# EnricoMiccoli/nodal

Measured on AMD Instinct MI355X. Metric: circuits_per_sec, higher is better.
Workload: dtype f64; 1 GPU; cfg3: grid(1000) 1e6 nodes, sparse CSR path; n=999999, nnz=4995995, parallelism=one GPU

## Files before the change

### nodal_amd/csrc/knobs.h

```cpp
#pragma once
#include <stdint.h>
#include <stdlib.h>

#include <optional>

namespace knob {

struct Present {
    const char *name;
    bool now() const { return getenv(name) != nullptr; }
};
struct OnUnless0 {
    const char *name;
    bool now() const { const char *e = getenv(name); return !(e && atoi(e) == 0); }
};
struct OffUnlessNon0 {
    const char *name;
    bool now() const { const char *e = getenv(name); return e && atoi(e) != 0; }
};
struct OnIfSet0 {
    const char *name;
    bool now() const { const char *e = getenv(name); return e != nullptr && atoi(e) == 0; }
};
struct Level {
    const char *name;
    int now() const {
        const char *e = getenv(name);
        if (!e) return 0;
        const int v = atoi(e);
        return v > 1 ? v : 1;
    }
};
struct Int {
    const char *name;
    int dflt;
    int now() const { const char *e = getenv(name); return e ? atoi(e) : dflt; }
};
struct Int64 {
    const char *name;
    int64_t dflt;
    int64_t now() const { const char *e = getenv(name); return e ? atoll(e) : dflt; }
};
struct Double {
    const char *name;
    double dflt;
    double now() const { const char *e = getenv(name); return e ? atof(e) : dflt; }
};
struct IntIfSet {
    const char *name;
    std::optional<int> now() const { const char *e = getenv(name); return e ? std::optional<int>(atoi(e)) : std::nullopt; }
};
struct Int64IfSet {
    const char *name;
    std::optional<int64_t> now() const { const char *e = getenv(name); return e ? std::optional<int64_t>(atoll(e)) : std::nullopt; }
};
struct DoubleIfSet {
    const char *name;
    std::optional<double> now() const { const char *e = getenv(name); return e ? std::optional<double>(atof(e)) : std::nullopt; }
};
struct Text {
    const char *name;
    const char *now() const { return getenv(name); }
};

inline constexpr Present TRACE{"NODAL_TRACE"};
inline constexpr Level POISON{"NODAL_POISON"};
inline constexpr Present NOFILL{"NODAL_NOFILL"};
inline constexpr Present NANCHECK{"NODAL_NANCHECK"};
inline constexpr Double WAIT_TIMEOUT_S{"NODAL_WAIT_TIMEOUT_S", 60.0};
inline constexpr Text STREAM_PRIORITY{"NODAL_STREAM_PRIORITY"};
inline constexpr IntIfSet EXTRA_STREAMS{"NODAL_EXTRA_STREAMS"};
inline constexpr IntIfSet HOST_THREADS{"NODAL_HOST_THREADS"};
inline constexpr IntIfSet CSV_CHUNKS{"NODAL_CSV_CHUNKS"};
inline constexpr OnUnless0 FOLD_STREAM{"NODAL_FOLD_STREAM"};
inline constexpr OffUnlessNon0 COUNT_LDS{"NODAL_COUNT_LDS"};
inline constexpr IntIfSet DENSE_BLOCKINV{"NODAL_DENSE_BLOCKINV"};
inline constexpr IntIfSet GJ_SCALAR{"NODAL_GJ_SCALAR"};
inline constexpr OnUnless0 GJ_DPP{"NODAL_GJ_DPP"};
inline constexpr OnUnless0 BI_SYM{"NODAL_BI_SYM"};
inline constexpr OnIfSet0 BI_MASKED{"NODAL_BI_MASKED"};
inline constexpr Int PANEL_CUS{"NODAL_PANEL_CUS", 32};
inline constexpr Int64 BI_UNMASK_ROWS{"NODAL_BI_UNMASK_ROWS", 0};
inline constexpr OnUnless0 BI_EARLY_COPY{"NODAL_BI_EARLY_COPY"};
inline constexpr Int BI_FIRST_BLOCKS{"NODAL_BI_FIRST_BLOCKS", 2};
inline constexpr Text BI_SWITCH{"NODAL_BI_SWITCH"};
inline constexpr Text BI_SWITCH2{"NODAL_BI_SWITCH2"};
inline constexpr Text BI_WIDTH{"NODAL_BI_WIDTH"};
inline constexpr IntIfSet GEPP_PANEL{"NODAL_GEPP_PANEL"};
inline constexpr Int GEPP_MAX{"NODAL_GEPP_MAX", 1280};
inline constexpr Present GEPP_PROBE{"NODAL_GEPP_PROBE"};
inline constexpr Int64IfSet FCG_MAXIT{"NODAL_FCG_MAXIT"};
inline constexpr OnUnless0 FCG_HOST_SUM{"NODAL_FCG_HOST_SUM"};
inline constexpr Double FCG_LOOK{"NODAL_FCG_LOOK", 0.75};
inline constexpr OnUnless0 LOWDEG{"NODAL_LOWDEG"};
inline constexpr IntIfSet LOWDEG_SHARE{"NODAL_LOWDEG_SHARE"};
inline constexpr Int64 LOWDEG_MIN{"NODAL_LOWDEG_MIN", 32};
inline constexpr Present SPARSE_FORCE_DIRECT{"NODAL_SPARSE_FORCE_DIRECT"};
inline constexpr Present SPARSE_CHILD_DIRECT{"NODAL_SPARSE_CHILD_DIRECT"};
inline constexpr OnUnless0 SAGG{"NODAL_SAGG"};
inline constexpr OnUnless0 SA_REUSE{"NODAL_SA_REUSE"};
inline constexpr OnUnless0 SA_FORK{"NODAL_SA_FORK"};
inline constexpr Double SA_SPREAD{"NODAL_SA_SPREAD", 16.0};
inline constexpr Double SA_SHARE{"NODAL_SA_SHARE", 0.9};
inline constexpr IntIfSet SA_MIS{"NODAL_SA_MIS"};
inline constexpr Text SA_OMEGA_P{"NODAL_SA_OMEGA_P"};
inline constexpr Double SA_PADSLACK{"NODAL_SA_PADSLACK", 1.3};
inline constexpr OnUnless0 SA_D16{"NODAL_SA_D16"};
inline constexpr Int SA_GG{"NODAL_SA_GG", 40};
inline constexpr Int64 SA_GCAP{"NODAL_SA_GCAP", 16384};
inline constexpr Int SA_GROWS{"NODAL_SA_GROWS", 4};
inline constexpr OnUnless0 SA_GDYN{"NODAL_SA_GDYN"};
inline constexpr Int SA_GLIST{"NODAL_SA_GLIST", 1024};
inline constexpr Int SA_GSEG{"NODAL_SA_GSEG", 4};
inline constexpr Text SA_NU{"NODAL_SA_NU"};
inline constexpr Int SA_KCYCLE{"NODAL_SA_KCYCLE", 1};
inline constexpr Int SA_KLEVELS{"NODAL_SA_KLEVELS", 1};
inline constexpr OnUnless0 SA_KFREEZE{"NODAL_SA_KFREEZE"};
inline constexpr OnUnless0 SA_FUSE_DIR{"NODAL_SA_FUSE_DIR"};
inline constexpr OffUnlessNon0 SA_GRAPH{"NODAL_SA_GRAPH"};
inline constexpr Text SA_FOLD_POST{"NODAL_SA_FOLD_POST"};
inline constexpr OffUnlessNon0 SA_FOLD_CHECK{"NODAL_SA_FOLD_CHECK"};
inline constexpr OnUnless0 SA_FOLD_VISIT{"NODAL_SA_FOLD_VISIT"};
inline constexpr Int64 SA_VISIT_CAP{"NODAL_SA_VISIT_CAP", 16777216};
inline constexpr OffUnlessNon0 SA_VISIT_CHECK{"NODAL_SA_VISIT_CHECK"};
inline constexpr OnUnless0 SA_RESTRICT_B{"NODAL_SA_RESTRICT_B"};
inline constexpr OffUnlessNon0 SA_RESTRICT_CHECK{"NODAL_SA_RESTRICT_CHECK"};
inline constexpr OnUnless0 SA_TAIL_DENSE{"NODAL_SA_TAIL_DENSE"};
inline constexpr OffUnlessNon0 SA_TAIL_CHECK{"NODAL_SA_TAIL_CHECK"};
inline constexpr Int SA_TAIL_NU{"NODAL_SA_TAIL_NU", 3};
inline constexpr Present TAIL_PROBE{"NODAL_TAIL_PROBE"};
inline constexpr IntIfSet AMG_PASSES0{"NODAL_AMG_PASSES0"};
inline constexpr IntIfSet AMG_PASSES1{"NODAL_AMG_PASSES1"};
inline constexpr IntIfSet AMG_SWEEPS0{"NODAL_AMG_SWEEPS0"};
inline constexpr IntIfSet AMG_BLOCK{"NODAL_AMG_BLOCK"};
inline constexpr DoubleIfSet AMG_THETA{"NODAL_AMG_THETA"};
inline constexpr Present AMG_KEEP_DENSE{"NODAL_AMG_KEEP_DENSE"};
inline constexpr Present AMG_NOTAIL{"NODAL_AMG_NOTAIL"};
inline constexpr IntIfSet AMG_KMAX{"NODAL_AMG_KMAX"};
inline constexpr OnUnless0 PAIRS_BLOCK{"NODAL_PAIRS_BLOCK"};
inline constexpr OnUnless0 PAIRS_FUNCTIONAL{"NODAL_PAIRS_FUNCTIONAL"};
inline constexpr Int PAIRS_DIRECT{"NODAL_PAIRS_DIRECT", -1};
inline constexpr Int64 PAIRS_DIRECT_MIN{"NODAL_PAIRS_DIRECT_MIN", 256};
inline constexpr Double MULTI_BAR{"NODAL_MULTI_BAR", 1e-14};
inline constexpr IntIfSet PRESOLVE{"NODAL_PRESOLVE"};
inline constexpr OnUnless0 PRESOLVE_KEEP{"NODAL_PRESOLVE_KEEP"};
inline constexpr IntIfSet FGMRES_WINDOW{"NODAL_FGMRES_WINDOW"};
inline constexpr Text DIRECT_NB{"NODAL_DIRECT_NB"};
inline constexpr Int DIRECT_LANES{"NODAL_DIRECT_LANES", 4};
inline constexpr DoubleIfSet DIRECT_MAX_GB{"NODAL_DIRECT_MAX_GB"};
inline constexpr IntIfSet DIRECT_BIG_DIM{"NODAL_DIRECT_BIG_DIM"};
inline constexpr OnUnless0 DIRECT_FRONT_LDS{"NODAL_DIRECT_FRONT_LDS"};
inline constexpr Int DIRECT_LDS_BS{"NODAL_DIRECT_LDS_BS", 64};
inline constexpr OnUnless0 DIRECT_PANEL_REGS{"NODAL_DIRECT_PANEL_REGS"};
inline constexpr OnUnless0 DIRECT_BATCHED{"NODAL_DIRECT_BATCHED"};
inline constexpr OnUnless0 DIRECT_WAVE{"NODAL_DIRECT_WAVE"};
inline constexpr Present DIRECT_LEVELS{"NODAL_DIRECT_LEVELS"};
inline constexpr OnUnless0 DIRECT_SUPER{"NODAL_DIRECT_SUPER"};
inline constexpr OnUnless0 DIRECT_APPLY_STEPPED{"NODAL_DIRECT_APPLY_STEPPED"};
inline constexpr OnUnless0 DIRECT_PEEL{"NODAL_DIRECT_PEEL"};
inline constexpr Int ND_DEPTH{"NODAL_ND_DEPTH", 4};
inline constexpr Int64 ND_PAR{"NODAL_ND_PAR", 20000};
inline constexpr Present SLU_DEBUG{"SLU_DEBUG"};

}
```

### nodal_amd/csrc/sagg.hip

```cpp
#include <hip/hip_ext.h>

#include <atomic>
#include <type_traits>

#include "galerkin_groups.h"
#include "group.h"

int grounded_flags(nodal_ctx *h, uint8_t *flags_dev);

namespace {

using grp::TB;
constexpr int PW = 4;
constexpr int ACAP = 64;
constexpr int RCAP = 96;
constexpr int RCAP_SMALL = 512;
constexpr int RCAP_SMALL_ROWS = 16384;
inline int rcap_for(int64_t nc) { return nc <= RCAP_SMALL_ROWS ? RCAP_SMALL : RCAP; }
constexpr int W0_MAX = 32;
constexpr int COARSEST = 64;
constexpr int MAX_LEVELS = 12;
constexpr int MIS_ROUNDS = 6;
constexpr int TAIL_MAX_N = 1024;
constexpr int TAIL_LEVELS = 6;
constexpr int TAIL_LDS_BUDGET = 150 * 1024;
constexpr int APAD = 32;
constexpr int DOT_BLOCKS = 1024;
#ifndef NODAL_SA_OMEGA
#define NODAL_SA_OMEGA 0.85
#endif
constexpr double OMEGA = NODAL_SA_OMEGA;
constexpr double OMEGA_P = 0.70;
constexpr double OMEGA_P_COARSE = 0.85;
using cyc_t = nodal_cyc_t;

inline unsigned grid_for(int64_t n, unsigned cap = 8192) {
    int64_t g = (n + TB - 1) / TB;
    if (g < 1) g = 1;
    if (g >= 64) g = (g + 7) & ~(int64_t)7;
    return (unsigned)(g > cap ? cap : g);
}
inline int64_t pad64(int64_t n) { return (n + 63) & ~(int64_t)63; }
inline size_t align256(size_t x) { return (x + 255) & ~(size_t)255; }

__device__ __forceinline__ unsigned xcd_block() {
    const unsigned g = gridDim.x, b = blockIdx.x;
    return (g & 7u) ? b : (b & 7u) * (g >> 3) + (b >> 3);
}


struct Ell {
    int64_t n = 0, ld = 0;
    int32_t width = 0;
    const int32_t *col = nullptr;
    const int16_t *dcol = nullptr;
    const double *val = nullptr;
    const float *valf = nullptr;
    const int32_t *len = nullptr;
};

enum { ST_MAXLEN = 0, ST_GRADED = 1, ST_BADDIAG = 2, ST_OVERFLOW = 3, ST_NNZ = 4, ST_UNASSIGNED = 5,
       ST_MAXR = 6, ST_NC = 7 ,
       ST_FARCOL = 8 ,
       ST_FOLDMISS = 9 ,
       ST_VISITMISS = 10 ,
       ST_RESTRICTMISS = 11 ,
       ST_COUNT = 12 };

struct SLevel {
    int64_t n = 0, ld = 0, nc = 0;
    int32_t width = 0;
    int32_t maxlen = 0;
    int32_t wfix = 0;
    int64_t nnz = 0;
    DevBuf acol, aval, alen, dinv;
    DevBuf adcol;
    bool d16 = false;
    DevBuf agg, pcol, pval;
    DevBuf rcol, rval, rlen;
    int64_t rld = 0;
    DevBuf vec, part, gflag;
    DevBuf avalf, pvalf, rvalf;
    DevBuf wcol, wval, wlen;
    int32_t wslots = 0;
    bool fold_want = false, fold = false;
    DevBuf p2col, p2val, p2len, d2;
    bool visit_want = false, visit = false;
    DevBuf wtstart, wtcol, wtval, wtsrc;
// ... 132 lines not shown
        m = max(m, bstat[i]);
        t += bstat[BSTAT_MAX + i];
    }
    atomicMax(&s_max, m);
    atomicAdd(&s_sum, t);
    __syncthreads();
    if (threadIdx.x == 0) {
        if (slot_max >= 0) stats[slot_max] = s_max;
        if (slot_sum >= 0) stats[slot_sum] = s_sum;
    }
}

__global__ __launch_bounds__(TB) void row_stats(int64_t n, const int32_t *__restrict__ indptr,
                                                const int32_t *__restrict__ indices,
                                                const double *__restrict__ data, double share, double spread,
                                                bool general, unsigned long long *__restrict__ stats,
                                                uint32_t *__restrict__ bstat) {
    int32_t mlen = 0;
    uint32_t graded = 0, bad = 0, far = 0;
    for (int64_t i = (int64_t)xcd_block() * TB + threadIdx.x; i < n; i += (int64_t)gridDim.x * TB) {
        const int32_t e0 = indptr[i], e1 = indptr[i + 1];
        mlen = max(mlen, e1 - e0);
        double d = 0.0, mx = 0.0, mn = 1e300;
        for (int32_t e = e0; e < e1; ++e) {
            const double v = data[e];
            const int64_t dc = (int64_t)indices[e] - i;
            if (dc > 32767 || dc < -32767) far = 1;
            if (indices[e] == (int32_t)i) d = v;
            else if (v != 0.0) {
                mx = fmax(mx, fabs(v));
                mn = fmin(mn, fabs(v));
                if (v > 0.0 && !general) bad = 1;
            }
        }
        if (!(d > 0.0)) bad = 1;
        graded += (d > 0.0 && (mx > share * d || mx > spread * mn)) ? 1u : 0u;
    }
    __shared__ unsigned int s_len, s_graded, s_bad;
    if (threadIdx.x == 0) s_len = s_graded = s_bad = 0;
    __syncthreads();
    atomicMax(&s_len, (unsigned)mlen);
    if (graded) atomicAdd(&s_graded, graded);
    if (bad) atomicOr(&s_bad, 1u);
    if (far) atomicOr(&s_bad, 2u);
    __syncthreads();
    if (threadIdx.x == 0) {
        bstat[blockIdx.x] = s_len;
        bstat[BSTAT_MAX + blockIdx.x] = s_graded;
        if (s_bad & 1u) atomicOr(&stats[ST_BADDIAG], 1ull);
        if (s_bad & 2u) stats[ST_FARCOL] = 1ull;
    }
}

__global__ __launch_bounds__(TB) void csr_to_ell(int64_t n, int64_t ld, const int32_t *__restrict__ indptr,
                                                 const int32_t *__restrict__ indices,
                                                 const double *__restrict__ data, int32_t *__restrict__ col,
                                                 double *__restrict__ val, float *__restrict__ valf,
                                                 int32_t *__restrict__ len, double *__restrict__ dinv, int32_t wpad,
                                                 int16_t *__restrict__ dcol) {
    for (int64_t i = (int64_t)xcd_block() * TB + threadIdx.x; i < n; i += (int64_t)gridDim.x * TB) {
        const int32_t e0 = indptr[i], e1 = indptr[i + 1];
        double d = 1.0;
        for (int32_t e = e0; e < e1; ++e) {
            const int32_t c = indices[e];
            const double v = data[e];
            col[(int64_t)(e - e0) * ld + i] = c;
            if (dcol) dcol[(int64_t)(e - e0) * ld + i] = (int16_t)(c - (int32_t)i);
            val[(int64_t)(e - e0) * ld + i] = v;
            valf[(int64_t)(e - e0) * ld + i] = (float)v;
            if (c == (int32_t)i) d = v;
        }
        for (int32_t s = e1 - e0; s < wpad; ++s) {
            col[(int64_t)s * ld + i] = (int32_t)i;
            if (dcol) dcol[(int64_t)s * ld + i] = 0;
            val[(int64_t)s * ld + i] = 0.0;
            valf[(int64_t)s * ld + i] = 0.0f;
        }
        len[i] = e1 - e0;
        dinv[i] = 1.0 / d;
    }
}


__device__ __forceinline__ uint32_t hash30(uint32_t x) {
    x ^= x >> 16;
    x *= 0x7feb352du;
    x ^= x >> 15;
    x *= 0x846ca68bu;
    x ^= x >> 16;
    return x & 0x3fffffffu;
}

__global__ __launch_bounds__(TB) void mis_init(int64_t n, uint32_t *__restrict__ T) {
    for (int64_t i = (int64_t)xcd_block() * TB + threadIdx.x; i < n; i += (int64_t)gridDim.x * TB)
        T[i] = (1u << 30) | hash30((uint32_t)i);
}

template <int NB>
__device__ __forceinline__ uint32_t nbr_max_batch(const Ell &A, const uint32_t *__restrict__ v, int64_t i, int32_t l, int32_t s0,
                                                  uint32_t best) {
    int32_t c[NB];
#pragma unroll
    for (int u = 0; u < NB; ++u) c[u] = A.col[(int64_t)(s0 + u < l ? s0 + u : 0) * A.ld + i];
    uint32_t t[NB];
#pragma unroll
    for (int u = 0; u < NB; ++u) t[u] = v[c[u]];
#pragma unroll
    for (int u = 0; u < NB; ++u) best = t[u] > best ? t[u] : best;
    return best;
}
__device__ __forceinline__ uint32_t nbr_max(const Ell &A, const uint32_t *__restrict__ v, int64_t i, int32_t l, uint32_t best) {
    if (l <= 5) return nbr_max_batch<5>(A, v, i, l, 0, best);
    for (int32_t s0 = 0; s0 < l; s0 += 8) best = nbr_max_batch<8>(A, v, i, l, s0, best);
    return best;
}

__global__ __launch_bounds__(TB) void mis_max(Ell A, const uint32_t *__restrict__ v, uint32_t *__restrict__ m) {
    for (int64_t i = (int64_t)xcd_block() * TB + threadIdx.x; i < A.n; i += (int64_t)gridDim.x * TB)
        m[i] = nbr_max(A, v, i, A.len[i], v[i]);
}

__global__ __launch_bounds__(TB) void mis_update(Ell A, uint32_t *__restrict__ T, const uint32_t *__restrict__ m1) {
    for (int64_t i = (int64_t)xcd_block() * TB + threadIdx.x; i < A.n; i += (int64_t)gridDim.x * TB) {
        const uint32_t own = T[i];
        if ((own >> 30) != 1) continue;
        const uint32_t best = nbr_max(A, m1, i, A.len[i], m1[i]);
        if (best == own) T[i] = own | (2u << 30);
        else if ((best >> 30) == 3) T[i] = 0;
    }
}

__global__ __launch_bounds__(TB) void mis_count(int64_t n, const uint32_t *__restrict__ T,
                                                unsigned long long *__restrict__ out) {
    uint32_t left = 0;
    for (int64_t i = (int64_t)xcd_block() * TB + threadIdx.x; i < n; i += (int64_t)gridDim.x * TB)
        left += (T[i] >> 30) == 1 ? 1u : 0u;
#pragma unroll
    for (int off = 32; off > 0; off >>= 1) left += __shfl_down(left, off, 64);
    if ((threadIdx.x & 63) == 0 && left) atomicAdd(out, (unsigned long long)left);
}

__global__ __launch_bounds__(TB) void mis_flag_roots(Ell A, const uint32_t *__restrict__ T,
                                                     uint32_t *__restrict__ flag) {
    for (int64_t i = (int64_t)xcd_block() * TB + threadIdx.x; i <= A.n; i += (int64_t)gridDim.x * TB) {
        uint32_t f = 0;
        if (i < A.n) {
            const uint32_t own = T[i];
            if ((own >> 30) == 3) f = 1;
            else if ((own >> 30) == 1) {
                bool near = false;
                const int32_t l = A.len[i];
                for (int32_t s = 0; s < l; ++s) near = near || (T[A.col[(int64_t)s * A.ld + i]] >> 30) == 3;
                f = near ? 0u : 1u;
            }
        }
        flag[i] = f;
    }
}

constexpr int64_t MIS_SMALL_MAX = 1024;
__global__ __launch_bounds__(1024) void mis_small(Ell A, uint32_t *__restrict__ T, uint32_t *__restrict__ M,
                                                  uint32_t *__restrict__ flag, int rounds) {
    const int64_t n = A.n;
    for (int64_t i = threadIdx.x; i < n; i += 1024) T[i] = (1u << 30) | hash30((uint32_t)i);
    __syncthreads();
    for (int r = 0; r < rounds; ++r) {
        for (int64_t i = threadIdx.x; i < n; i += 1024) {
            uint32_t best = T[i];
            const int32_t l = A.len[i];
            for (int32_t s = 0; s < l; ++s) {
                const uint32_t t = T[A.col[(int64_t)s * A.ld + i]];
                best = t > best ? t : best;
            }
            M[i] = best;
        }
        __syncthreads();
        for (int64_t i = threadIdx.x; i < n; i += 1024) {
            const uint32_t own = T[i];
            if ((own >> 30) != 1) continue;
            uint32_t best = M[i];
            const int32_t l = A.len[i];
            for (int32_t s = 0; s < l; ++s) {
                const uint32_t t = M[A.col[(int64_t)s * A.ld + i]];
                best = t > best ? t : best;
            }
            if (best == own) T[i] = own | (2u << 30);
            else if ((best >> 30) == 3) T[i] = 0;
        }
        __syncthreads();
    }
    for (int64_t i = threadIdx.x; i <= n; i += 1024) {
        uint32_t f = 0;
        if (i < n) {
            const uint32_t own = T[i];
            if ((own >> 30) == 3) f = 1;
            else if ((own >> 30) == 1) {
                bool near = false;
                const int32_t l = A.len[i];
                for (int32_t s = 0; s < l; ++s) near = near || (T[A.col[(int64_t)s * A.ld + i]] >> 30) == 3;
                f = near ? 0u : 1u;
            }
        }
        flag[i] = f;
    }
}

__global__ __launch_bounds__(TB) void assign_near(Ell A, const uint32_t *__restrict__ T,
                                                  const uint32_t *__restrict__ flag,
                                                  const uint32_t *__restrict__ id, int32_t *__restrict__ agg1) {
    for (int64_t i = (int64_t)xcd_block() * TB + threadIdx.x; i < A.n; i += (int64_t)gridDim.x * TB) {
        int32_t a = -1;
        if (flag[i]) a = (int32_t)id[i];
        else {
            uint32_t best = 0;
            const int32_t l = A.len[i];
            auto batch = [&](auto NBc, int32_t s0) {
                constexpr int NB = decltype(NBc)::value;
                int32_t c[NB];
#pragma unroll
                for (int u = 0; u < NB; ++u) c[u] = A.col[(int64_t)(s0 + u < l ? s0 + u : 0) * A.ld + i];
                uint32_t fl[NB], tt[NB], idd[NB];
#pragma unroll
                for (int u = 0; u < NB; ++u) {
                    fl[u] = flag[c[u]];
                    tt[u] = T[c[u]];
                    idd[u] = id[c[u]];
                }
#pragma unroll
                for (int u = 0; u < NB; ++u) {
                    if (s0 + u >= l || c[u] == (int32_t)i || !fl[u]) continue;
                    const uint32_t t = tt[u] | (3u << 30);
                    if (t > best) { best = t; a = (int32_t)idd[u]; }
                }
            };
            if (l <= 5) batch(std::integral_constant<int, 5>{}, 0);
            else for (int32_t s0 = 0; s0 < l; s0 += 8) batch(std::integral_constant<int, 8>{}, s0);
        }
        agg1[i] = a;
    }
}

__global__ __launch_bounds__(TB) void assign_far(Ell A, const int32_t *__restrict__ agg1, int32_t *__restrict__ agg,
                                                 unsigned long long *__restrict__ stats) {
    for (int64_t i = (int64_t)xcd_block() * TB + threadIdx.x; i < A.n; i += (int64_t)gridDim.x * TB) {
        int32_t a = agg1[i];
        if (a < 0) {
            double bw = -1.0;
            const int32_t l = A.len[i];
            auto batch = [&](auto NBc, int32_t s0) {
                constexpr int NB = decltype(NBc)::value;
                int32_t c[NB];
                double w[NB];
#pragma unroll
                for (int u = 0; u < NB; ++u) {
                    const int64_t at = (int64_t)(s0 + u < l ? s0 + u : 0) * A.ld + i;
                    c[u] = A.col[at];
                    w[u] = fabs(A.val[at]);
                }
                int32_t aj[NB];
#pragma unroll
                for (int u = 0; u < NB; ++u) aj[u] = agg1[c[u]];
#pragma unroll
                for (int u = 0; u < NB; ++u) {
                    if (s0 + u >= l || c[u] == (int32_t)i || aj[u] < 0) continue;
                    if (w[u] > bw) { bw = w[u]; a = aj[u]; }
                }
            };
            if (l <= 5) batch(std::integral_constant<int, 5>{}, 0);
            else for (int32_t s0 = 0; s0 < l; s0 += 8) batch(std::integral_constant<int, 8>{}, s0);
            if (a < 0) stats[ST_UNASSIGNED] = 1;
        }
        agg[i] = a;
    }
}

__global__ __launch_bounds__(TB) void build_P(Ell A, const double *__restrict__ dinv,
                                              const int32_t *__restrict__ agg, int32_t *__restrict__ pcol,
                                              double *__restrict__ pval, float *__restrict__ pvalf, double omega_p) {
    for (int64_t i = (int64_t)xcd_block() * TB + threadIdx.x; i < A.n; i += (int64_t)gridDim.x * TB) {
        int32_t c[PW];
        double v[PW];
#pragma unroll
        for (int k = 0; k < PW; ++k) { c[k] = -1; v[k] = 0.0; }
        const int32_t own = agg[i];
        c[0] = own;
        v[0] = 1.0;
        const double wd = omega_p * dinv[i];
        const int32_t l = A.len[i];
        for (int32_t s = 0; s < l; ++s) {
            const int32_t J = agg[A.col[(int64_t)s * A.ld + i]];
            const double t = -wd * A.val[(int64_t)s * A.ld + i];
            bool placed = false;
#pragma unroll
            for (int k = 0; k < PW; ++k) {
                if (!placed && c[k] == J) { v[k] += t; placed = true; }
            }
#pragma unroll
            for (int k = 1; k < PW; ++k) {
                if (!placed && c[k] < 0) { c[k] = J; v[k] = t; placed = true; }
            }
            if (!placed) v[0] += t;
        }
#pragma unroll
        for (int k = 0; k < PW; ++k) {
            pcol[(int64_t)k * A.ld + i] = c[k];
            pval[(int64_t)k * A.ld + i] = v[k];
            pvalf[(int64_t)k * A.ld + i] = (float)v[k];
        }
    }
}

template <bool LEN>
struct TKey { static constexpr int SHIFT = LEN ? 6 : 2; };
template <bool LEN = false>
__global__ __launch_bounds__(TB) void r_count(int64_t n, int64_t ld, const int32_t *__restrict__ pcol,
                                              uint32_t *__restrict__ cnt, uint32_t *__restrict__ place,
                                              const int32_t *__restrict__ len = nullptr) {
    for (int64_t i = (int64_t)xcd_block() * TB + threadIdx.x; i < n; i += (int64_t)gridDim.x * TB) {
        if constexpr (LEN) {
            const int32_t m = len[i];
            for (int32_t k = 0; k < m; ++k)
                place[(int64_t)k * ld + i] = atomicAdd(&cnt[pcol[(int64_t)k * ld + i]], 1u);
        } else {
#pragma unroll
            for (int k = 0; k < PW; ++k) {
                const int32_t J = pcol[(int64_t)k * ld + i];
                if (J >= 0) place[(int64_t)k * ld + i] = atomicAdd(&cnt[J], 1u);
            }
        }
    }
}
template <bool LEN = false>
__global__ __launch_bounds__(TB) void r_fill(int64_t n, int64_t ld, const int32_t *__restrict__ pcol,
                                             const uint32_t *__restrict__ rstart, const uint32_t *__restrict__ place,
                                             uint64_t *__restrict__ keys, const int32_t *__restrict__ len = nullptr,
                                             uint32_t keycap = 0, int64_t nc = 0) {
    if constexpr (LEN) {
        if (rstart[nc] > keycap) return;
    }
    for (int64_t i = (int64_t)xcd_block() * TB + threadIdx.x; i < n; i += (int64_t)gridDim.x * TB) {
        if constexpr (LEN) {
            const int32_t m = len[i];
            for (int32_t k = 0; k < m; ++k)
                keys[rstart[pcol[(int64_t)k * ld + i]] + place[(int64_t)k * ld + i]] =
                    ((uint64_t)i << TKey<true>::SHIFT) | (uint64_t)k;
        } else {
#pragma unroll
            for (int k = 0; k < PW; ++k) {
                const int32_t J = pcol[(int64_t)k * ld + i];
                if (J >= 0) keys[rstart[J] + place[(int64_t)k * ld + i]] = ((uint64_t)i << 2) | (uint64_t)k;
            }
        }
    }
}
__global__ __launch_bounds__(TB) void r_to_ell(int64_t nc, int64_t rld, const uint32_t *__restrict__ rstart,
// ... 904 lines not shown
        return f;
    }();
    return s;
}
bool fold_wanted(int level, int64_t n) {
    if (level > 0 && n <= TAIL_MAX_N) return false;
    const FoldSetting &f = fold_setting();
    switch (f.mode) {
    case 1: return false;
    case 2: return true;
    case 3: return (f.mask >> level & 1u) != 0;
    default: return n <= FOLD_MAX_ROWS;
    }
}
void decide_folds(SHierarchy *H, const unsigned long long *hs, bool trace) {
    for (int k = 0; k < H->nlev; ++k) {
        SLevel *L = H->pool[k];
        const bool runs_cycle = k + 1 < H->nlev && (H->tail < 0 || k < H->tail);
        const bool miss = hs[(size_t)k * ST_COUNT + ST_FOLDMISS] != 0;
        L->fold = L->fold_want && runs_cycle && !miss;
        if (trace && L->fold_want && runs_cycle)
            fprintf(stderr, "[sagg] level %d (%lld rows): first post-smoothing sweep %s\n", k, (long long)L->n,
                    miss ? "NOT folded: a row of A P lacks a column of its P row (no stored diagonal)"
                         : "folded into the prolongation");
        const bool wide = hs[(size_t)k * ST_COUNT + ST_VISITMISS] != 0;
        L->visit = L->visit_want && L->fold && !wide;
        if (trace && L->visit_want)
            fprintf(stderr, "[sagg] level %d (%lld rows): visit %s\n", k, (long long)L->n,
                    L->visit ? "in three launches" : "NOT in three launches: W missing, or a row of P2 beyond its slots");
        const unsigned long long over = hs[(size_t)k * ST_COUNT + ST_RESTRICTMISS] |
                                        (H->sym_valid ? H->sym_stats[(size_t)k * ST_COUNT + ST_RESTRICTMISS] : 0ull);
        L->restrict_b = L->restrict_want && L->fold && !L->visit && !over;
        if (trace && L->restrict_want && runs_cycle)
            fprintf(stderr, "[sagg] level %d (%lld rows): restriction %s\n", k, (long long)L->n,
                    L->restrict_b ? "from b beside the residual launch"
                                  : over ? "NOT from b: a row of W^T beyond the per-row sort, or more entries than its arrays hold"
                                         : "NOT from b: W missing, or the level visits in three launches");
    }
}

void apply_nu_knob(SHierarchy *H);
constexpr int WT_AVG = 16;
bool restrict_wanted(SHierarchy *H, int l, const SLevel *L) {
    static const bool on = knob::SA_RESTRICT_B.now();
    if (!on || l < 1 || H->general || !L->fold_want || (int64_t)L->wslots * L->ld >= (1ll << 31)) return false;
    apply_nu_knob(H);
    return H->nu[l < 2 ? l : 2] == 1;
}
int reserve_wt(nodal_ctx *h, SHierarchy *H, SLevel *L, int64_t nc) {
    const int64_t cap = (int64_t)(L->wslots < WT_AVG ? L->wslots : WT_AVG) * L->n;
    L->wtcap = cap;
    NODAL_HIP_TRY(h, L->wtstart.reserve(align256((size_t)(nc + 1) * 4) + 256));
    NODAL_HIP_TRY(h, L->wtcol.reserve((size_t)cap * 4 + 64));
    NODAL_HIP_TRY(h, L->wtval.reserve((size_t)cap * 4 + 64));
    NODAL_HIP_TRY(h, L->wtsrc.reserve((size_t)cap * 4 + 64));
    NODAL_HIP_TRY(h, H->wt_keys.reserve((size_t)cap * 8 + 64));
    NODAL_HIP_TRY(h, H->wt_scratch.reserve(align256(scan_tmp_bytes(nc + 1)) + (size_t)L->wslots * L->ld * 4 + 64));
    return NODAL_OK;
}
int build_wt(nodal_ctx *h, SHierarchy *H, int l) {
    hipStream_t st = h->stream;
    SLevel *L = H->pool[l];
    const int64_t n = L->n, ld = L->ld, nc = L->nc;
    const uint32_t cap = (uint32_t)L->wtcap;
    uint32_t *wtstart = L->wtstart.as<uint32_t>();
    char *sc = H->wt_scratch.as<char>();
    uint32_t *place = reinterpret_cast<uint32_t *>(sc + align256(scan_tmp_bytes(nc + 1)));
    uint64_t *keys = H->wt_keys.as<uint64_t>();
    const int32_t *wcol = L->wcol.as<int32_t>(), *wlen = L->wlen.as<int32_t>();
    NODAL_HIP_TRY(h, hipMemsetAsync(wtstart, 0, align256((size_t)(nc + 1) * 4) + 256, st));
    r_count<true><<<grid_for(n), TB, 0, st>>>(n, ld, wcol, wtstart, place, wlen);
    NODAL_HIP_TRY(h, hipGetLastError());
    NODAL_TRY(scan_exclusive_u32(h, wtstart, wtstart, nc + 1, nullptr, sc));
    r_fill<true><<<grid_for(n), TB, 0, st>>>(n, ld, wcol, wtstart, place, keys, wlen, cap, nc);
    r_sort_short<<<grid_for(nc), TB, 0, st>>>(wtstart, keys, nc, cap);
    r_sort_medium<<<(unsigned)(nc < 8192 ? nc : 8192), 64, 0, st>>>(wtstart, keys, nc, cap);
    wt_pack<<<grid_for(nc * 64), TB, 0, st>>>(nc, wtstart, keys, ld, L->wval.as<float>(), cap, L->wtcol.as<int32_t>(),
                                             L->wtval.as<float>(), L->wtsrc.as<int32_t>(),
                                             H->stats.as<unsigned long long>() + (size_t)l * ST_COUNT);
    NODAL_HIP_TRY(h, hipGetLastError());
    return NODAL_OK;
}

int build_level(nodal_ctx *h, SHierarchy *H, int l, unsigned long long *hs, bool *declined, bool *stop) {
    hipStream_t st = h->stream;
    SLevel *L = H->level(l);
    const int64_t n = L->n, ld = L->ld;
    Ell A = L->A();
    A.width = L->maxlen;
    unsigned long long *dstats = H->stats.as<unsigned long long>();

    NODAL_HIP_TRY(h, H->mis_t.reserve((size_t)n * 8 + 64));
    NODAL_HIP_TRY(h, H->mis_m.reserve((size_t)n * 8 + 64));
    NODAL_HIP_TRY(h, H->mis_flag.reserve((size_t)(n + 1) * 4 + 64));
    NODAL_HIP_TRY(h, H->mis_id.reserve((size_t)(n + 1) * 4 + 64 + scan_tmp_bytes(n + 1)));
    NODAL_HIP_TRY(h, H->agg1.reserve((size_t)n * 4 + 64));
    NODAL_HIP_TRY(h, L->agg.reserve((size_t)n * 4 + 64));
    NODAL_HIP_TRY(h, H->cursor.reserve((MIS_ROUNDS + 2) * 8 + 64));
    uint32_t *T = H->mis_t.as<uint32_t>(), *M = H->mis_m.as<uint32_t>();
    uint32_t *flag = H->mis_flag.as<uint32_t>(), *id = H->mis_id.as<uint32_t>();
    unsigned long long *cnt = H->cursor.as<unsigned long long>();
    void *scan_tmp = H->mis_id.as<char>() + (((size_t)(n + 1) * 4 + 63) & ~(size_t)63);

    const unsigned g = grid_for(n);
    static const bool trace_mis = knob::TRACE.now();
    if (trace_mis) NODAL_HIP_TRY(h, hipMemsetAsync(cnt, 0, (MIS_ROUNDS + 2) * 8, st));
    static const int mis_rounds = std::min(MIS_ROUNDS, std::max(1, knob::SA_MIS.now().value_or(MIS_ROUNDS)));
    if (n <= MIS_SMALL_MAX && !trace_mis) {
        mis_small<<<1, 1024, 0, st>>>(A, T, M, flag, mis_rounds);
    } else {
        mis_init<<<g, TB, 0, st>>>(n, T);
        for (int r = 0; r < mis_rounds; ++r) {
            mis_max<<<g, TB, 0, st>>>(A, T, M);
            mis_update<<<g, TB, 0, st>>>(A, T, M);
            if (trace_mis) mis_count<<<g, TB, 0, st>>>(n, T, cnt + r + 1);
        }
        mis_flag_roots<<<grid_for(n + 1), TB, 0, st>>>(A, T, flag);
    }
    NODAL_HIP_TRY(h, hipGetLastError());
    NODAL_TRY(scan_exclusive_u32(h, flag, id, n + 1, reinterpret_cast<uint32_t *>(dstats + (size_t)l * ST_COUNT + ST_NC),
                                 scan_tmp));
    NODAL_HIP_TRY(h, hipMemcpyAsync(hs, dstats, (size_t)MAX_LEVELS * ST_COUNT * 8, hipMemcpyDeviceToHost, st));
    unsigned long long hcnt[MIS_ROUNDS + 1] = {0};
    if (trace_mis) NODAL_HIP_TRY(h, hipMemcpyAsync(hcnt, cnt, sizeof hcnt, hipMemcpyDeviceToHost, st));
    if (!H->ev_copy) NODAL_HIP_TRY(h, hipEventCreateWithFlags(&H->ev_copy, hipEventDisableTiming));
    NODAL_HIP_TRY(h, hipEventRecord(H->ev_copy, st));
    NODAL_HIP_TRY(h, L->pcol.reserve((size_t)PW * ld * 4 + 64));
    NODAL_HIP_TRY(h, L->pval.reserve((size_t)PW * ld * 8 + 64));
    NODAL_HIP_TRY(h, L->pvalf.reserve((size_t)PW * ld * 4 + 64));
    assign_near<<<g, TB, 0, st>>>(A, T, flag, id, H->agg1.as<int32_t>());
    assign_far<<<g, TB, 0, st>>>(A, H->agg1.as<int32_t>(), L->agg.as<int32_t>(), dstats + (size_t)l * ST_COUNT);
    build_P<<<g, TB, 0, st>>>(A, L->dinv.as<double>(), L->agg.as<int32_t>(), L->pcol.as<int32_t>(),
                             L->pval.as<double>(), L->pvalf.as<float>(), omega_p(l));
    NODAL_HIP_TRY(h, hipGetLastError());
    NODAL_WAIT_EVENT(h, H->ev_copy, st);
    if (trace_mis) {
        fprintf(stderr, "[sagg] level %d: undecided after each MIS round:", l);
        for (int r = 1; r <= MIS_ROUNDS; ++r) fprintf(stderr, " %llu", hcnt[r]);
        fprintf(stderr, "\n");
    }
    const int64_t nc = (int64_t)(hs[(size_t)l * ST_COUNT + ST_NC] & 0xffffffffull);
    if (l > 0) {
        const unsigned long long *s = hs + (size_t)l * ST_COUNT;
        L->maxlen = (int32_t)s[ST_MAXLEN];
        L->nnz = (int64_t)s[ST_NNZ];
        A.width = L->maxlen;
        if (s[ST_OVERFLOW] || s[ST_BADDIAG] || hs[(size_t)(l - 1) * ST_COUNT + ST_OVERFLOW] ||
            hs[(size_t)(l - 1) * ST_COUNT + ST_UNASSIGNED]) {
            *declined = true;
            return NODAL_OK;
        }
    }
    if (nc >= n || L->maxlen <= 1) {
        *stop = true;
        return NODAL_OK;
    }
    if ((nc * 2 > n && n > 4096) || nc < 1) {
        *declined = true;
        return NODAL_OK;
    }
    L->nc = nc;

    static const bool fork_allowed = knob::SA_FORK.now();
    if (H->aux && !nodal_extra_streams_ok(h) && nodal_calls_in_flight() <= 1) {
        NODAL_WAIT_STREAM(h, H->aux);
        (void)hipStreamDestroy(H->aux);
        H->aux = nullptr;
        H->aux_tried = false;
    }
    if (fork_allowed && !H->aux_tried && nodal_extra_streams_ok(h)) {
        H->aux_tried = true;
        if (hipStreamCreateWithFlags(&H->aux, hipStreamNonBlocking) != hipSuccess) H->aux = nullptr;
        if (H->aux && ((!H->ev_fork && hipEventCreateWithFlags(&H->ev_fork, hipEventDisableTiming) != hipSuccess) ||
                       (!H->ev_join && hipEventCreateWithFlags(&H->ev_join, hipEventDisableTiming) != hipSuccess) ||
                       (!H->ev_flags && hipEventCreateWithFlags(&H->ev_flags, hipEventDisableTiming) != hipSuccess) ||
                       (!H->ev_w && hipEventCreateWithFlags(&H->ev_w, hipEventDisableTiming) != hipSuccess) ||
                       (!H->ev_wt && hipEventCreateWithFlags(&H->ev_wt, hipEventDisableTiming) != hipSuccess))) {
            (void)hipStreamDestroy(H->aux);
            H->aux = nullptr;
        }
        (void)hipGetLastError();
    }
    const bool forked = fork_allowed && H->aux != nullptr && nodal_extra_streams_ok(h);
    const size_t a4 = (((size_t)(nc + 1) * 4) + 255) & ~(size_t)255;
    const size_t scan2 = (scan_tmp_bytes(nc + 1) + 255) & ~(size_t)255;
    NODAL_HIP_TRY(h, H->rstart.reserve(a4 + 256 + scan2 + (size_t)PW * ld * 4 + 64));
    NODAL_HIP_TRY(h, H->keys.reserve((size_t)PW * n * 8 + 64));
    SLevel *C = H->level(l + 1);
    C->n = nc;
    C->ld = pad64(nc);
    C->width = ACAP;
    C->nc = 0;
    L->rld = C->ld;
    const int rcap = rcap_for(nc);
    NODAL_HIP_TRY(h, L->rcol.reserve((size_t)rcap * C->ld * 4 + 64));
    NODAL_HIP_TRY(h, L->rval.reserve((size_t)rcap * C->ld * 8 + 64));
    NODAL_HIP_TRY(h, L->rvalf.reserve((size_t)rcap * C->ld * 4 + 64));
    NODAL_HIP_TRY(h, L->rlen.reserve((size_t)C->ld * 4 + 64));
    NODAL_HIP_TRY(h, C->acol.reserve((size_t)ACAP * C->ld * 4 + 64));
    NODAL_HIP_TRY(h, C->aval.reserve((size_t)ACAP * C->ld * 8 + 64));
    NODAL_HIP_TRY(h, C->avalf.reserve((size_t)ACAP * C->ld * 4 + 64));
    NODAL_HIP_TRY(h, C->alen.reserve((size_t)C->ld * 4 + 64));
    NODAL_HIP_TRY(h, C->dinv.reserve((size_t)C->ld * 8 + 64));
    if (forked && H->want_flags) {
        if (l == 0) NODAL_HIP_TRY(h, L->gflag.reserve((size_t)n + 64));
        NODAL_HIP_TRY(h, C->gflag.reserve((size_t)C->n + 64));
    }
    {
        const int apw = L->maxlen <= 6 ? 16 : 64;
        NODAL_HIP_TRY(h, H->apcol.reserve((size_t)apw * ld * 4 + 64));
        NODAL_HIP_TRY(h, H->apval.reserve((size_t)apw * ld * 8 + 64));
        NODAL_HIP_TRY(h, H->aplen.reserve((size_t)ld * 4 + 64));
        L->fold = false;
        L->fold_want = fold_wanted(l, n);
        L->wslots = apw;
        if (L->fold_want) {
            NODAL_HIP_TRY(h, L->wcol.reserve((size_t)apw * ld * 4 + 64));
            NODAL_HIP_TRY(h, L->wval.reserve((size_t)apw * ld * 4 + 64));
            NODAL_HIP_TRY(h, L->wlen.reserve((size_t)ld * 4 + 64));
        }
        L->restrict_b = false;
        L->restrict_want = restrict_wanted(H, l, L);
// ... 1414 lines not shown
```

Measured before the change: 182.7 circuits/s.

## Fuse MIS max/update rounds into one launch per round via recomputation

Moves the MIS rule logic into shared host/device templates and adds fused kernels that compute one round in a single launch. Each row recomputes its neighbours' closed-neighbourhood maxima rather than reading an intermediate array, and the round ping-pongs between two buffers. It is active by default only for level 0 when every row has at most five entries (the grid stencil); the lanes-per-row forms and the fused assignment are disabled by zero thresholds. The goal is to halve the kernel launches and the global round-trips per MIS round, at the cost of redundant two-hop gathers.

After: 180.4 circuits/s. -1.3%, worse.

```diff
diff --git a/nodal_amd/csrc/knobs.h b/nodal_amd/csrc/knobs.h
--- a/nodal_amd/csrc/knobs.h
+++ b/nodal_amd/csrc/knobs.h
@@ -103,6 +103,7 @@
 inline constexpr Double SA_SPREAD{"NODAL_SA_SPREAD", 16.0};
 inline constexpr Double SA_SHARE{"NODAL_SA_SHARE", 0.9};
 inline constexpr IntIfSet SA_MIS{"NODAL_SA_MIS"};
+inline constexpr Int SA_MIS_FUSED{"NODAL_SA_MIS_FUSED", 1};
 inline constexpr Text SA_OMEGA_P{"NODAL_SA_OMEGA_P"};
 inline constexpr Double SA_PADSLACK{"NODAL_SA_PADSLACK", 1.3};
 inline constexpr OnUnless0 SA_D16{"NODAL_SA_D16"};
diff --git a/nodal_amd/csrc/mis_rules.h b/nodal_amd/csrc/mis_rules.h
--- /dev/null
+++ b/nodal_amd/csrc/mis_rules.h
@@ -0,0 +1,134 @@
+#pragma once
+#include <stdint.h>
+
+#if defined(__HIPCC__) || defined(__CUDACC__)
+#define MIS_HD __host__ __device__ __forceinline__
+#else
+#define MIS_HD inline
+#endif
+
+template <int N>
+struct MisInt {
+    static constexpr int value = N;
+};
+
+MIS_HD uint32_t mis_hash30(uint32_t x) {
+    x ^= x >> 16;
+    x *= 0x7feb352du;
+    x ^= x >> 15;
+    x *= 0x846ca68bu;
+    x ^= x >> 16;
+    return x & 0x3fffffffu;
+}
+MIS_HD uint32_t mis_initial(uint32_t i) { return (1u << 30) | mis_hash30(i); }
+MIS_HD bool mis_undecided(uint32_t t) { return (t >> 30) == 1; }
+
+template <int NB, class Col, class Word>
+MIS_HD uint32_t mis_max_batch(int64_t i, int32_t l, int32_t s0, Col col, Word word, uint32_t best) {
+    int32_t c[NB];
+#pragma unroll
+    for (int u = 0; u < NB; ++u) c[u] = col(i, s0 + u < l ? s0 + u : 0);
+    uint32_t t[NB];
+#pragma unroll
+    for (int u = 0; u < NB; ++u) t[u] = word(c[u]);
+#pragma unroll
+    for (int u = 0; u < NB; ++u) best = t[u] > best ? t[u] : best;
+    return best;
+}
+
+template <bool SHORT, class Col, class Word>
+MIS_HD uint32_t mis_closed_max(int64_t i, int32_t l, Col col, Word word) {
+    const uint32_t own = word(i);
+    if (SHORT || l <= 5) return mis_max_batch<5>(i, l, 0, col, word, own);
+    uint32_t best = own;
+    for (int32_t s0 = 0; s0 < l; s0 += 8) best = mis_max_batch<8>(i, l, s0, col, word, best);
+    return best;
+}
+
+MIS_HD uint32_t mis_decide(uint32_t own, uint32_t best) {
+    if (best == own) return own | (2u << 30);
+    if ((best >> 30) == 3) return 0;
+    return own;
+}
+
+template <bool SHORT, class Col, class M1>
+MIS_HD uint32_t mis_round_row(int64_t i, int32_t l, uint32_t own, Col col, M1 m1) {
+    if (!mis_undecided(own)) return own;
+    return mis_decide(own, mis_closed_max<SHORT>(i, l, col, m1));
+}
+
+template <bool SHORT, class Col, class Flag, class Word, class Id>
+MIS_HD int32_t mis_near(int64_t i, int32_t l, Col col, Flag flag, Word word, Id id) {
+    if (flag(i)) return (int32_t)id(i);
+    int32_t a = -1;
+    uint32_t best = 0;
+    auto batch = [&](auto NBc, int32_t s0) {
+        constexpr int NB = decltype(NBc)::value;
+        int32_t c[NB];
+#pragma unroll
+        for (int u = 0; u < NB; ++u) c[u] = col(i, s0 + u < l ? s0 + u : 0);
+        uint32_t fl[NB], tt[NB], idd[NB];
+#pragma unroll
+        for (int u = 0; u < NB; ++u) {
+            fl[u] = flag(c[u]);
+            tt[u] = word(c[u]);
+            idd[u] = id(c[u]);
+        }
+#pragma unroll
+        for (int u = 0; u < NB; ++u) {
+            if (s0 + u >= l || c[u] == (int32_t)i || !fl[u]) continue;
+            const uint32_t t = tt[u] | (3u << 30);
+            if (t > best) { best = t; a = (int32_t)idd[u]; }
+        }
+    };
+    if (SHORT || l <= 5) batch(MisInt<5>{}, 0);
+    else for (int32_t s0 = 0; s0 < l; s0 += 8) batch(MisInt<8>{}, s0);
+    return a;
+}
+
+struct MisFar {
+    double w = -1.0;
+    int32_t slot = 0x7fffffff;
+    int32_t agg = -1;
+};
+MIS_HD void mis_far_take(MisFar &best, double w, int32_t slot, int32_t a) {
+    if (w > best.w || (w == best.w && slot < best.slot)) { best.w = w; best.slot = slot; best.agg = a; }
+}
+template <class Col, class Wt, class Near>
+MIS_HD MisFar mis_far_strided(int64_t i, int32_t l, int32_t s_first, int32_t s_step, Col col, Wt wt, Near near) {
+    MisFar best;
+    for (int32_t s = s_first; s < l; s += s_step) {
+        const int32_t c = col(i, s);
+        const double w = wt(i, s);
+        if (c == (int32_t)i) continue;
+        const int32_t a = near(c);
+        if (a >= 0) mis_far_take(best, w, s, a);
+    }
+    return best;
+}
+template <bool SHORT, class Col, class Wt, class Near>
+MIS_HD int32_t mis_far(int64_t i, int32_t l, Col col, Wt wt, Near near) {
+    MisFar best;
+    auto batch = [&](auto NBc, int32_t s0) {
+        constexpr int NB = decltype(NBc)::value;
+        int32_t c[NB];
+        double w[NB];
+#pragma unroll
+        for (int u = 0; u < NB; ++u) {
+            const int32_t s = s0 + u < l ? s0 + u : 0;
+            c[u] = col(i, s);
+            w[u] = wt(i, s);
+        }
+        int32_t aj[NB];
+#pragma unroll
+        for (int u = 0; u < NB; ++u) aj[u] = near(c[u]);
+#pragma unroll
+        for (int u = 0; u < NB; ++u) {
+            if (s0 + u >= l || c[u] == (int32_t)i || aj[u] < 0) continue;
+            mis_far_take(best, w[u], s0 + u, aj[u]);
+        }
+    };
+    if (SHORT || l <= 5) batch(MisInt<5>{}, 0);
+    else for (int32_t s0 = 0; s0 < l; s0 += 8) batch(MisInt<8>{}, s0);
+    return best.agg;
+}
diff --git a/nodal_amd/csrc/sagg.hip b/nodal_amd/csrc/sagg.hip
--- a/nodal_amd/csrc/sagg.hip
+++ b/nodal_amd/csrc/sagg.hip
@@ -4,6 +4,7 @@
 #include <type_traits>
 
 #include "galerkin_groups.h"
+#include "mis_rules.h"
 #include "group.h"
 
 int grounded_flags(nodal_ctx *h, uint8_t *flags_dev);
@@ -302,52 +303,94 @@
 }
 
 
-__device__ __forceinline__ uint32_t hash30(uint32_t x) {
-    x ^= x >> 16;
-    x *= 0x7feb352du;
-    x ^= x >> 15;
-    x *= 0x846ca68bu;
-    x ^= x >> 16;
-    return x & 0x3fffffffu;
-}
+struct EllCol {
+    const int32_t *__restrict__ col;
+    int64_t ld;
+    __device__ __forceinline__ int32_t operator()(int64_t i, int32_t s) const { return col[(int64_t)s * ld + i]; }
+};
+struct EllWeight {
+    const double *__restrict__ val;
+    int64_t ld;
+    __device__ __forceinline__ double operator()(int64_t i, int32_t s) const { return fabs(val[(int64_t)s * ld + i]); }
+};
+template <class V>
+struct ArrayOf {
+    const V *__restrict__ v;
+    __device__ __forceinline__ V operator()(int64_t k) const { return v[k]; }
+};
+struct InitialWord {
+    __device__ __forceinline__ uint32_t operator()(int64_t k) const { return mis_initial((uint32_t)k); }
+};
 
 __global__ __launch_bounds__(TB) void mis_init(int64_t n, uint32_t *__restrict__ T) {
     for (int64_t i = (int64_t)xcd_block() * TB + threadIdx.x; i < n; i += (int64_t)gridDim.x * TB)
-        T[i] = (1u << 30) | hash30((uint32_t)i);
-}
-
-template <int NB>
-__device__ __forceinline__ uint32_t nbr_max_batch(const Ell &A, const uint32_t *__restrict__ v, int64_t i, int32_t l, int32_t s0,
-                                                  uint32_t best) {
-    int32_t c[NB];
-#pragma unroll
-    for (int u = 0; u < NB; ++u) c[u] = A.col[(int64_t)(s0 + u < l ? s0 + u : 0) * A.ld + i];
-    uint32_t t[NB];
-#pragma unroll
-    for (int u = 0; u < NB; ++u) t[u] = v[c[u]];
-#pragma unroll
-    for (int u = 0; u < NB; ++u) best = t[u] > best ? t[u] : best;
-    return best;
-}
-__device__ __forceinline__ uint32_t nbr_max(const Ell &A, const uint32_t *__restrict__ v, int64_t i, int32_t l, uint32_t best) {
-    if (l <= 5) return nbr_max_batch<5>(A, v, i, l, 0, best);
-    for (int32_t s0 = 0; s0 < l; s0 += 8) best = nbr_max_batch<8>(A, v, i, l, s0, best);
-    return best;
+        T[i] = mis_initial((uint32_t)i);
 }
 
 __global__ __launch_bounds__(TB) void mis_max(Ell A, const uint32_t *__restrict__ v, uint32_t *__restrict__ m) {
     for (int64_t i = (int64_t)xcd_block() * TB + threadIdx.x; i < A.n; i += (int64_t)gridDim.x * TB)
-        m[i] = nbr_max(A, v, i, A.len[i], v[i]);
+        m[i] = mis_closed_max<false>(i, A.len[i], EllCol{A.col, A.ld}, ArrayOf<uint32_t>{v});
 }
 
 __global__ __launch_bounds__(TB) void mis_update(Ell A, uint32_t *__restrict__ T, const uint32_t *__restrict__ m1) {
     for (int64_t i = (int64_t)xcd_block() * TB + threadIdx.x; i < A.n; i += (int64_t)gridDim.x * TB) {
         const uint32_t own = T[i];
-        if ((own >> 30) != 1) continue;
-        const uint32_t best = nbr_max(A, m1, i, A.len[i], m1[i]);
-        if (best == own) T[i] = own | (2u << 30);
-        else if ((best >> 30) == 3) T[i] = 0;
-    }
+        if (!mis_undecided(own)) continue;
+        const uint32_t now = mis_round_row<false>(i, A.len[i], own, EllCol{A.col, A.ld}, ArrayOf<uint32_t>{m1});
+        if (now != own) T[i] = now;
+    }
+}
+
+template <bool FIRST>
+__global__ __launch_bounds__(TB) void mis_round_short(Ell A, const uint32_t *__restrict__ T_old,
+                                                      uint32_t *__restrict__ T_new) {
+    const EllCol col{A.col, A.ld};
+    const ArrayOf<int32_t> len{A.len};
+    for (int64_t i = (int64_t)xcd_block() * TB + threadIdx.x; i < A.n; i += (int64_t)gridDim.x * TB) {
+        if constexpr (FIRST) {
+            const InitialWord word;
+            auto m1 = [&](int64_t j) { return mis_closed_max<true>(j, len(j), col, word); };
+            T_new[i] = mis_round_row<true>(i, len(i), word(i), col, m1);
+        } else {
+            const ArrayOf<uint32_t> word{T_old};
+            auto m1 = [&](int64_t j) { return mis_closed_max<true>(j, len(j), col, word); };
+            T_new[i] = mis_round_row<true>(i, len(i), word(i), col, m1);
+        }
+    }
+}
+
+constexpr int MIS_LPR = 16;
+template <bool FIRST, class Word>
+__device__ __forceinline__ void mis_round_lanes_body(const Ell &A, Word word, uint32_t *__restrict__ T_new) {
+    const EllCol col{A.col, A.ld};
+    const int32_t q = (int32_t)(threadIdx.x % MIS_LPR);
+    constexpr int ROWS = TB / MIS_LPR;
+    for (int64_t i = (int64_t)xcd_block() * ROWS + threadIdx.x / MIS_LPR; i < A.n; i += (int64_t)gridDim.x * ROWS) {
+        const uint32_t own = word(i);
+        uint32_t now = own;
+        if (mis_undecided(own)) {
+            const int32_t l = A.len[i];
+            uint32_t best = own;
+            for (int32_t s = q - 1; s < l; s += MIS_LPR) {
+                const int64_t j = s < 0 ? i : (int64_t)col(i, s);
+                const uint32_t m = mis_closed_max<false>(j, A.len[j], col, word);
+                best = m > best ? m : best;
+            }
+#pragma unroll
+            for (int off = 1; off < MIS_LPR; off <<= 1) {
+                const uint32_t other = __shfl_xor(best, off, 64);
+                best = other > best ? other : best;
+            }
+            now = mis_decide(own, best);
+        }
+        if (q == 0) T_new[i] = now;
+    }
+}
+template <bool FIRST>
+__global__ __launch_bounds__(TB) void mis_round_lanes(Ell A, const uint32_t *__restrict__ T_old,
+                                                      uint32_t *__restrict__ T_new) {
+    if constexpr (FIRST) mis_round_lanes_body<FIRST>(A, InitialWord{}, T_new);
+    else mis_round_lanes_body<FIRST>(A, ArrayOf<uint32_t>{T_old}, T_new);
 }
 
 __global__ __launch_bounds__(TB) void mis_count(int64_t n, const uint32_t *__restrict__ T,
@@ -382,7 +425,7 @@
 __global__ __launch_bounds__(1024) void mis_small(Ell A, uint32_t *__restrict__ T, uint32_t *__restrict__ M,
                                                   uint32_t *__restrict__ flag, int rounds) {
     const int64_t n = A.n;
-    for (int64_t i = threadIdx.x; i < n; i += 1024) T[i] = (1u << 30) | hash30((uint32_t)i);
+    for (int64_t i = threadIdx.x; i < n; i += 1024) T[i] = mis_initial((uint32_t)i);
     __syncthreads();
     for (int r = 0; r < rounds; ++r) {
         for (int64_t i = threadIdx.x; i < n; i += 1024) {
@@ -428,36 +471,9 @@
 __global__ __launch_bounds__(TB) void assign_near(Ell A, const uint32_t *__restrict__ T,
                                                   const uint32_t *__restrict__ flag,
                                                   const uint32_t *__restrict__ id, int32_t *__restrict__ agg1) {
-    for (int64_t i = (int64_t)xcd_block() * TB + threadIdx.x; i < A.n; i += (int64_t)gridDim.x * TB) {
-        int32_t a = -1;
-        if (flag[i]) a = (int32_t)id[i];
-        else {
-            uint32_t best = 0;
-            const int32_t l = A.len[i];
-            auto batch = [&](auto NBc, int32_t s0) {
-                constexpr int NB = decltype(NBc)::value;
-                int32_t c[NB];
-#pragma unroll
-                for (int u = 0; u < NB; ++u) c[u] = A.col[(int64_t)(s0 + u < l ? s0 + u : 0) * A.ld + i];
-                uint32_t fl[NB], tt[NB], idd[NB];
-#pragma unroll
-                for (int u = 0; u < NB; ++u) {
-                    fl[u] = flag[c[u]];
-                    tt[u] = T[c[u]];
-                    idd[u] = id[c[u]];
-                }
-#pragma unroll
-                for (int u = 0; u < NB; ++u) {
-                    if (s0 + u >= l || c[u] == (int32_t)i || !fl[u]) continue;
-                    const uint32_t t = tt[u] | (3u << 30);
-                    if (t > best) { best = t; a = (int32_t)idd[u]; }
-                }
-            };
-            if (l <= 5) batch(std::integral_constant<int, 5>{}, 0);
-            else for (int32_t s0 = 0; s0 < l; s0 += 8) batch(std::integral_constant<int, 8>{}, s0);
-        }
-        agg1[i] = a;
-    }
+    for (int64_t i = (int64_t)xcd_block() * TB + threadIdx.x; i < A.n; i += (int64_t)gridDim.x * TB)
+        agg1[i] = mis_near<false>(i, A.len[i], EllCol{A.col, A.ld}, ArrayOf<uint32_t>{flag}, ArrayOf<uint32_t>{T},
+                                  ArrayOf<uint32_t>{id});
 }
 
 __global__ __launch_bounds__(TB) void assign_far(Ell A, const int32_t *__restrict__ agg1, int32_t *__restrict__ agg,
@@ -465,32 +481,52 @@
     for (int64_t i = (int64_t)xcd_block() * TB + threadIdx.x; i < A.n; i += (int64_t)gridDim.x * TB) {
         int32_t a = agg1[i];
         if (a < 0) {
-            double bw = -1.0;
-            const int32_t l = A.len[i];
-            auto batch = [&](auto NBc, int32_t s0) {
-                constexpr int NB = decltype(NBc)::value;
-                int32_t c[NB];
-                double w[NB];
-#pragma unroll
-                for (int u = 0; u < NB; ++u) {
-                    const int64_t at = (int64_t)(s0 + u < l ? s0 + u : 0) * A.ld + i;
-                    c[u] = A.col[at];
-                    w[u] = fabs(A.val[at]);
-                }
-                int32_t aj[NB];
-#pragma unroll
-                for (int u = 0; u < NB; ++u) aj[u] = agg1[c[u]];
-#pragma unroll
-                for (int u = 0; u < NB; ++u) {
-                    if (s0 + u >= l || c[u] == (int32_t)i || aj[u] < 0) continue;
-                    if (w[u] > bw) { bw = w[u]; a = aj[u]; }
-                }
-            };
-            if (l <= 5) batch(std::integral_constant<int, 5>{}, 0);
-            else for (int32_t s0 = 0; s0 < l; s0 += 8) batch(std::integral_constant<int, 8>{}, s0);
+            a = mis_far<false>(i, A.len[i], EllCol{A.col, A.ld}, EllWeight{A.val, A.ld}, ArrayOf<int32_t>{agg1});
             if (a < 0) stats[ST_UNASSIGNED] = 1;
         }
         agg[i] = a;
+    }
+}
+
+__global__ __launch_bounds__(TB) void assign_short(Ell A, const uint32_t *__restrict__ T,
+                                                   const uint32_t *__restrict__ flag, const uint32_t *__restrict__ id,
+                                                   int32_t *__restrict__ agg, unsigned long long *__restrict__ stats) {
+    const EllCol col{A.col, A.ld};
+    const ArrayOf<uint32_t> fl{flag}, word{T}, ids{id};
+    for (int64_t i = (int64_t)xcd_block() * TB + threadIdx.x; i < A.n; i += (int64_t)gridDim.x * TB) {
+        int32_t a = mis_near<true>(i, A.len[i], col, fl, word, ids);
+        if (a < 0) {
+            auto near = [&](int64_t j) { return mis_near<true>(j, A.len[j], col, fl, word, ids); };
+            a = mis_far<true>(i, A.len[i], col, EllWeight{A.val, A.ld}, near);
+            if (a < 0) stats[ST_UNASSIGNED] = 1;
+        }
+        agg[i] = a;
+    }
+}
+
+__global__ __launch_bounds__(TB) void assign_lanes(Ell A, const uint32_t *__restrict__ T,
+                                                   const uint32_t *__restrict__ flag, const uint32_t *__restrict__ id,
+                                                   int32_t *__restrict__ agg, unsigned long long *__restrict__ stats) {
+    const EllCol col{A.col, A.ld};
+    const ArrayOf<uint32_t> fl{flag}, word{T}, ids{id};
+    const int32_t q = (int32_t)(threadIdx.x % MIS_LPR);
+    constexpr int ROWS = TB / MIS_LPR;
+    for (int64_t i = (int64_t)xcd_block() * ROWS + threadIdx.x / MIS_LPR; i < A.n; i += (int64_t)gridDim.x * ROWS) {
+        const int32_t l = A.len[i];
+        int32_t a = mis_near<false>(i, l, col, fl, word, ids);
+        if (a < 0) {
+            auto near = [&](int64_t j) { return mis_near<false>(j, A.len[j], col, fl, word, ids); };
+            MisFar best = mis_far_strided(i, l, q, MIS_LPR, col, EllWeight{A.val, A.ld}, near);
+#pragma unroll
+            for (int off = 1; off < MIS_LPR; off <<= 1) {
+                const double ow = __shfl_xor(best.w, off, 64);
+                const int32_t os = __shfl_xor(best.slot, off, 64), oa = __shfl_xor(best.agg, off, 64);
+                mis_far_take(best, ow, os, oa);
+            }
+            a = best.agg;
+            if (a < 0 && q == 0) stats[ST_UNASSIGNED] = 1;
+        }
+        if (q == 0) agg[i] = a;
     }
 }
 
@@ -1561,6 +1597,22 @@
     return NODAL_OK;
 }
 
+enum class MisForm { Pair, Short, Lanes };
+constexpr int64_t MIS_FUSED_SHORT_ROWS = INT64_MAX;
+constexpr int64_t MIS_FUSED_LANES_ROWS = 0;
+constexpr int64_t ASSIGN_FUSED_SHORT_ROWS = 0;
+constexpr int64_t ASSIGN_FUSED_LANES_ROWS = 0;
+MisForm mis_fused_form(int l, int64_t n, int32_t maxlen, int64_t short_rows, int64_t lanes_rows) {
+    static const int mode = knob::SA_MIS_FUSED.now();
+    if (mode == 0) return MisForm::Pair;
+    if (mode >= 2) short_rows = lanes_rows = INT64_MAX;
+    if (l == 0 && maxlen <= 5) return n <= short_rows ? MisForm::Short : MisForm::Pair;
+    return n <= lanes_rows ? MisForm::Lanes : MisForm::Pair;
+}
+const char *mis_form_name(MisForm f) {
+    return f == MisForm::Pair ? "two launches" : f == MisForm::Short ? "one launch (a thread per row)" : "one launch (lanes per row)";
+}
+
 int build_level(nodal_ctx *h, SHierarchy *H, int l, unsigned long long *hs, bool *declined, bool *stop) {
     hipStream_t st = h->stream;
     SLevel *L = H->level(l);
@@ -1573,7 +1625,9 @@
     NODAL_HIP_TRY(h, H->mis_m.reserve((size_t)n * 8 + 64));
     NODAL_HIP_TRY(h, H->mis_flag.reserve((size_t)(n + 1) * 4 + 64));
     NODAL_HIP_TRY(h, H->mis_id.reserve((size_t)(n + 1) * 4 + 64 + scan_tmp_bytes(n + 1)));
-    NODAL_HIP_TRY(h, H->agg1.reserve((size_t)n * 4 + 64));
+    const MisForm round_form = mis_fused_form(l, n, L->maxlen, MIS_FUSED_SHORT_ROWS, MIS_FUSED_LANES_ROWS);
+    const MisForm assign_form = mis_fused_form(l, n, L->maxlen, ASSIGN_FUSED_SHORT_ROWS, ASSIGN_FUSED_LANES_ROWS);
+    if (assign_form == MisForm::Pair) NODAL_HIP_TRY(h, H->agg1.reserve((size_t)n * 4 + 64));
     NODAL_HIP_TRY(h, L->agg.reserve((size_t)n * 4 + 64));
     NODAL_HIP_TRY(h, H->cursor.reserve((MIS_ROUNDS + 2) * 8 + 64));
     uint32_t *T = H->mis_t.as<uint32_t>(), *M = H->mis_m.as<uint32_t>();
@@ -1585,13 +1639,28 @@
     static const bool trace_mis = knob::TRACE.now();
     if (trace_mis) NODAL_HIP_TRY(h, hipMemsetAsync(cnt, 0, (MIS_ROUNDS + 2) * 8, st));
     static const int mis_rounds = std::min(MIS_ROUNDS, std::max(1, knob::SA_MIS.now().value_or(MIS_ROUNDS)));
-    if (n <= MIS_SMALL_MAX && !trace_mis) {
+    const bool small = n <= MIS_SMALL_MAX && !trace_mis;
+    if (small) {
         mis_small<<<1, 1024, 0, st>>>(A, T, M, flag, mis_rounds);
-    } else {
+    } else if (round_form == MisForm::Pair) {
         mis_init<<<g, TB, 0, st>>>(n, T);
         for (int r = 0; r < mis_rounds; ++r) {
             mis_max<<<g, TB, 0, st>>>(A, T, M);
             mis_update<<<g, TB, 0, st>>>(A, T, M);
+            if (trace_mis) mis_count<<<g, TB, 0, st>>>(n, T, cnt + r + 1);
+        }
+        mis_flag_roots<<<grid_for(n + 1), TB, 0, st>>>(A, T, flag);
+    } else {
+        const unsigned gl = grid_for(n * MIS_LPR);
+        for (int r = 0; r < mis_rounds; ++r) {
+            if (round_form == MisForm::Short) {
+                if (r == 0) mis_round_short<true><<<g, TB, 0, st>>>(A, T, M);
+                else mis_round_short<false><<<g, TB, 0, st>>>(A, T, M);
+            } else {
+                if (r == 0) mis_round_lanes<true><<<gl, TB, 0, st>>>(A, T, M);
+                else mis_round_lanes<false><<<gl, TB, 0, st>>>(A, T, M);
+            }
+            std::swap(T, M);
             if (trace_mis) mis_count<<<g, TB, 0, st>>>(n, T, cnt + r + 1);
         }
         mis_flag_roots<<<grid_for(n + 1), TB, 0, st>>>(A, T, flag);
@@ -1607,8 +1676,14 @@
     NODAL_HIP_TRY(h, L->pcol.reserve((size_t)PW * ld * 4 + 64));
     NODAL_HIP_TRY(h, L->pval.reserve((size_t)PW * ld * 8 + 64));
     NODAL_HIP_TRY(h, L->pvalf.reserve((size_t)PW * ld * 4 + 64));
-    assign_near<<<g, TB, 0, st>>>(A, T, flag, id, H->agg1.as<int32_t>());
-    assign_far<<<g, TB, 0, st>>>(A, H->agg1.as<int32_t>(), L->agg.as<int32_t>(), dstats + (size_t)l * ST_COUNT);
+    if (assign_form == MisForm::Pair) {
+        assign_near<<<g, TB, 0, st>>>(A, T, flag, id, H->agg1.as<int32_t>());
+        assign_far<<<g, TB, 0, st>>>(A, H->agg1.as<int32_t>(), L->agg.as<int32_t>(), dstats + (size_t)l * ST_COUNT);
+    } else if (assign_form == MisForm::Short) {
+        assign_short<<<g, TB, 0, st>>>(A, T, flag, id, L->agg.as<int32_t>(), dstats + (size_t)l * ST_COUNT);
+    } else {
+        assign_lanes<<<grid_for(n * MIS_LPR), TB, 0, st>>>(A, T, flag, id, L->agg.as<int32_t>(), dstats + (size_t)l * ST_COUNT);
+    }
     build_P<<<g, TB, 0, st>>>(A, L->dinv.as<double>(), L->agg.as<int32_t>(), L->pcol.as<int32_t>(),
                              L->pval.as<double>(), L->pvalf.as<float>(), omega_p(l));
     NODAL_HIP_TRY(h, hipGetLastError());
@@ -1617,6 +1692,8 @@
         fprintf(stderr, "[sagg] level %d: undecided after each MIS round:", l);
         for (int r = 1; r <= MIS_ROUNDS; ++r) fprintf(stderr, " %llu", hcnt[r]);
         fprintf(stderr, "\n");
+        fprintf(stderr, "[sagg] level %d: independent set by %s, assignment by %s\n", l,
+                mis_form_name(round_form), mis_form_name(assign_form));
     }
     const int64_t nc = (int64_t)(hs[(size_t)l * ST_COUNT + ST_NC] & 0xffffffffull);
     if (l > 0) {
```
